# leo-stan/torch-points3d

Hardware: AMD Instinct MI355X
Metric: point-clouds/sec fwd+bwd PointNet++SSG B=32 N=16384 (higher is better)
Workload: dtype f32; 1 GPU; PointNet++ SSG (unet_3_ss) train step fwd+bwd+Adam, B=32 per GPU, N=16384, FEAT=3, 10 classes, pos~U[-1,1]^3 (BASELINE configs[1]); launch=hip-graph replay; geometry of step i+1 on a 2nd stream during step i, global_batch=32, points=16384, parallelism=dp1, whole clouds per rank, one flat gradient all-reduce (RCCL) per step

## Files before the change

### torch_points3d_amd/csrc/rows.hip

```cpp
#include "tp3d_common.h"

namespace tp3d {

constexpr int RW_BLOCK = 256;

__global__ __launch_bounds__(RW_BLOCK) void group_concat_fwd_kernel(const float *__restrict__ pos,
                                                                     const float *__restrict__ new_pos,
                                                                     const float *__restrict__ x_cl,
                                                                     const int64_t *__restrict__ idx, int N, int np,
                                                                     int ns, int C, int ld, float radius,
                                                                     int normalize, int64_t total,
                                                                     float *__restrict__ out)
{
    const int Cw = C + 3;
    for (int64_t e = (int64_t)blockIdx.x * RW_BLOCK + threadIdx.x; e < total; e += (int64_t)gridDim.x * RW_BLOCK) {
        const int64_t row = e / ld;
        const int c = (int)(e - row * ld);
        if (c >= Cw) {
            out[e] = 0.0f;
            continue;
        }
        const int64_t bj = row / ns;
        const int b = (int)(bj / np);
        const int k = min(max((int)idx[row], 0), N - 1);
        float v;
        if (c < 3) {
            v = pos[((size_t)b * N + k) * 3 + c] - new_pos[bj * 3 + c];
            if (normalize) v = v / radius;
        } else {
            v = x_cl[((size_t)b * N + k) * C + (c - 3)];
        }
        out[e] = v;
    }
}

struct __attribute__((packed, aligned(4))) f4u {
    float v[4];
};
__global__ __launch_bounds__(RW_BLOCK) void group_concat_fwd4_kernel(const float *__restrict__ pos,
                                                                      const float *__restrict__ new_pos,
                                                                      const float *__restrict__ x_cl,
                                                                      const int64_t *__restrict__ idx, int N, int np,
                                                                      int ns, int C, int ld, float radius,
                                                                      int normalize, int64_t total4,
                                                                      float *__restrict__ out)
{
    const int Cw = C + 3, q = ld >> 2;
    for (int64_t e4 = (int64_t)blockIdx.x * RW_BLOCK + threadIdx.x; e4 < total4; e4 += (int64_t)gridDim.x * RW_BLOCK) {
        const int64_t row = e4 / q;
        const int c = (int)(e4 - row * q) * 4;
        const int64_t bj = row / ns;
        const int b = (int)(bj / np);
        const int k = min(max((int)idx[row], 0), N - 1);
        float t[4];
        if (c == 0) {
#pragma unroll
            for (int j = 0; j < 3; ++j) {
                float v = pos[((size_t)b * N + k) * 3 + j] - new_pos[bj * 3 + j];
                if (normalize) v = v / radius;
                t[j] = v;
            }
            t[3] = C > 0 ? x_cl[((size_t)b * N + k) * C] : 0.0f;
        } else if (c + 3 < Cw) {
            const f4u f = *reinterpret_cast<const f4u *>(x_cl + ((size_t)b * N + k) * C + (c - 3));
#pragma unroll
            for (int j = 0; j < 4; ++j) t[j] = f.v[j];
        } else {
#pragma unroll
            for (int j = 0; j < 4; ++j) t[j] = (c + j < Cw) ? x_cl[((size_t)b * N + k) * C + (c + j - 3)] : 0.0f;
        }
        *reinterpret_cast<float4 *>(out + e4 * 4) = make_float4(t[0], t[1], t[2], t[3]);
    }
}

constexpr int ST_ROWS = 256;
constexpr int ST_ROWS_SMALL = 32;
constexpr int64_t ST_SMALL_BELOW = 131072;
static inline int stat_rows(int64_t R) { return R >= ST_SMALL_BELOW ? ST_ROWS : ST_ROWS_SMALL; }

struct StatTile {
    int colthreads, rowlanes, gridx;
};
static inline StatTile stat_tile(int C, int V)
{
    int cols = (C + V - 1) / V;
    int ct = 1;
    while (ct < cols && ct < 64) ct <<= 1;
    StatTile t;
    t.colthreads = ct;
    t.rowlanes = RW_BLOCK / ct;
    t.gridx = (cols + ct - 1) / ct;
    return t;
}

template <int V, int MODE>
__global__ __launch_bounds__(RW_BLOCK) void colreduce_partial_kernel(
    const float *__restrict__ Y, const float *__restrict__ dA, const float *__restrict__ scale,
    const float *__restrict__ shift, const float *__restrict__ mean, const float *__restrict__ invstd, float slope,
    int64_t M, int C, int colthreads, int chunk_rows, float *__restrict__ partial , int reverse = 0)
{
    __shared__ float s1[RW_BLOCK * V], s2[RW_BLOCK * V];
    const int ct = threadIdx.x % colthreads, rl = threadIdx.x / colthreads;
    const int rowlanes = RW_BLOCK / colthreads;
    const int c = (blockIdx.x * colthreads + ct) * V;
    const int chunk = (MODE == 1 && reverse) ? (int)(gridDim.y - 1 - blockIdx.y) : (int)blockIdx.y;
    const int64_t r0 = (int64_t)chunk * chunk_rows;
    const int64_t r1 = min(r0 + chunk_rows, M);
    float a[V], q[V], sc[V], sh[V], mu[V], is[V];
#pragma unroll
    for (int v = 0; v < V; ++v) {
        a[v] = 0.0f;
        q[v] = 0.0f;
        if (MODE == 0) mu[v] = (c + v < C && r0 < M) ? Y[r0 * C + c + v] : 0.0f;
        if (MODE == 1 && c + v < C) {
            sc[v] = scale[c + v];
            sh[v] = shift[c + v];
            mu[v] = mean[c + v];
            is[v] = invstd[c + v];
        }
    }
    if (c < C) {
        constexpr int U = 4;
        for (int64_t r = r0 + rl; r < r1; r += (int64_t)rowlanes * U) {
            float y[U][V], d[U][V];
// ... 234 lines not shown
            o.y = leaky((y.y - mu.y) * sc.y + sh.y, slope);
            o.z = leaky((y.z - mu.z) * sc.z + sh.z, slope);
            o.w = leaky((y.w - mu.w) * sc.w + sh.w, slope);
            *reinterpret_cast<float4 *>(out + e) = o;
        } else {
            out[e] = leaky((Y[e] - mean[cw.c]) * scale[cw.c] + shift[cw.c], slope);
        }
    }
}

__global__ __launch_bounds__(RW_BLOCK) void bn_act_maxpool_kernel(const float *__restrict__ Y,
                                                                   const float *__restrict__ mean,
                                                                   const float *__restrict__ scale,
                                                                   const float *__restrict__ shift, float slope,
                                                                   int64_t G, int ns, int C,
                                                                   float *__restrict__ out, int *__restrict__ arg)
{
    const int64_t total = G * C;
    for (int64_t e = (int64_t)blockIdx.x * RW_BLOCK + threadIdx.x; e < total; e += (int64_t)gridDim.x * RW_BLOCK) {
        const int64_t g = e / C;
        const int c = (int)(e - g * C);
        const float mu = mean[c], sc = scale[c], sh = shift[c];
        const float *y = Y + (size_t)g * ns * C + c;
        float best = -INFINITY;
        int bs = 0;
        int s = 0;
        auto take = [&](float a, int row) {
            const bool is_nan = (__float_as_uint(a) & 0x7fffffffu) > 0x7f800000u;
            const bool have_nan = (__float_as_uint(best) & 0x7fffffffu) > 0x7f800000u;
            if (!have_nan && (is_nan || a > best)) {
                best = a;
                bs = row;
            }
        };
        for (; s + 8 <= ns; s += 8) {
            float v[8];
#pragma unroll
            for (int u = 0; u < 8; ++u) v[u] = y[(size_t)(s + u) * C];
#pragma unroll
            for (int u = 0; u < 8; ++u) {
                const float z = (v[u] - mu) * sc + sh;
                take(z > 0.0f ? z : z * slope, s + u);
            }
        }
        for (; s < ns; ++s) {
            const float z = (y[(size_t)s * C] - mu) * sc + sh;
            take(z > 0.0f ? z : z * slope, s);
        }
        out[e] = best;
        arg[e] = bs;
    }
}

__global__ __launch_bounds__(RW_BLOCK) void bn_pool_bwd_partial_kernel(const float *__restrict__ dP,
                                                                        const int *__restrict__ arg,
                                                                        const float *__restrict__ Y,
                                                                        const float *__restrict__ scale,
                                                                        const float *__restrict__ shift,
                                                                        const float *__restrict__ mean,
                                                                        const float *__restrict__ invstd, float slope,
                                                                        int64_t G, int ns, int C, int chunk_rows,
                                                                        float *__restrict__ partial)
{
    __shared__ float s1[4][64], s2[4][64];
    const int tc = threadIdx.x & 63, tr = threadIdx.x >> 6;
    const int c = blockIdx.x * 64 + tc;
    const int64_t g0 = (int64_t)blockIdx.y * chunk_rows;
    const int64_t g1 = min(g0 + chunk_rows, G);
    float a = 0.0f, q = 0.0f;
    if (c < C) {
        const float sc = scale[c], sh = shift[c], mu = mean[c], is = invstd[c];
        for (int64_t g = g0 + tr; g < g1; g += 4) {
            const int s = arg[g * C + c];
            const float y = Y[((size_t)g * ns + s) * C + c];
            const float z = (y - mu) * sc + sh;
            const float dz = dP[g * C + c] * (z > 0.0f ? 1.0f : slope);
            a += dz;
            q += dz * ((y - mu) * is);
        }
    }
    s1[tr][tc] = a;
    s2[tr][tc] = q;
    __syncthreads();
    if (tr == 0 && c < C) {
        a = (s1[0][tc] + s1[1][tc]) + (s1[2][tc] + s1[3][tc]);
        q = (s2[0][tc] + s2[1][tc]) + (s2[2][tc] + s2[3][tc]);
        partial[((size_t)blockIdx.y * 2 + 0) * C + c] = a;
        partial[((size_t)blockIdx.y * 2 + 1) * C + c] = q;
    }
}

__global__ __launch_bounds__(RW_BLOCK) void bn_bwd_finalize_kernel(const float *__restrict__ partial, int chunks,
                                                                    int C, float *__restrict__ dbeta,
                                                                    float *__restrict__ dgamma,
                                                                    const float *__restrict__ invstd, int64_t M,
                                                                    int training, float *__restrict__ c1,
                                                                    float *__restrict__ c2)
{
    double a, q;
    sum_partials(partial, chunks, C, blockIdx.x, a, q);
    if (threadIdx.x == 0) {
        dbeta[blockIdx.x] = (float)a;
        dgamma[blockIdx.x] = (float)q;
        if (c1) {
            const float invM = 1.0f / (float)M;
            c1[blockIdx.x] = training ? (float)a * invM : 0.0f;
            c2[blockIdx.x] = training ? invstd[blockIdx.x] * ((float)q * invM) : 0.0f;
        }
    }
}

__device__ __forceinline__ float bn_bwd_elem(float da, float y, float sc, float sh, float mu, float is, float db,
                                             float dg, float slope, float invM, int training)
{
    const float z = (y - mu) * sc + sh;
    const float dz = da * (z > 0.0f ? 1.0f : slope);
    float v = dz;
    if (training) v = dz - db * invM - ((y - mu) * is) * (dg * invM);
    return sc * v;
}

template <int V>
__global__ __launch_bounds__(RW_BLOCK) void bn_act_bwd_apply_kernel(
    const float *__restrict__ dA, const float *__restrict__ Y, const float *__restrict__ scale,
    const float *__restrict__ shift, const float *__restrict__ mean, const float *__restrict__ invstd,
    const float *__restrict__ dbeta, const float *__restrict__ dgamma, float slope, int64_t M, int C, int training,
    float *__restrict__ dY)
{
    const int64_t total = M * C;
    const float invM = 1.0f / (float)M;
    const int64_t stride = (int64_t)gridDim.x * RW_BLOCK * V;
// ... 69 lines not shown
        const size_t base = (size_t)g * ns * C + c;
        const int s_end = min(ns, (seg + 1) * seg_len);
        int s = seg * seg_len;
        for (; s + 8 <= s_end; s += 8) {
            float y[8];
#pragma unroll
            for (int u = 0; u < 8; ++u) y[u] = Y[base + (size_t)(s + u) * C];
#pragma unroll
            for (int u = 0; u < 8; ++u)
                dY[base + (size_t)(s + u) * C] =
                    bn_bwd_elem(s + u == sa ? dp : 0.0f, y[u], sc, sh, mu, is, db, dg, slope, invM, training);
        }
        for (; s < s_end; ++s) {
            const float y = Y[base + (size_t)s * C];
            dY[base + (size_t)s * C] = bn_bwd_elem(s == sa ? dp : 0.0f, y, sc, sh, mu, is, db, dg, slope, invM, training);
        }
    }
}

__global__ __launch_bounds__(RW_BLOCK) void interp_concat_fwd_kernel(const float *__restrict__ feat_cl,
                                                                      const int64_t *__restrict__ idx,
                                                                      const float *__restrict__ w,
                                                                      const float *__restrict__ skip_cl, int m, int n,
                                                                      int C1, int C2, int ld, int64_t total,
                                                                      float *__restrict__ out)
{
    const int Cw = C1 + C2;
    for (int64_t e = (int64_t)blockIdx.x * RW_BLOCK + threadIdx.x; e < total; e += (int64_t)gridDim.x * RW_BLOCK) {
        const int64_t row = e / ld;
        const int c = (int)(e - row * ld);
        if (c >= Cw) {
            out[e] = 0.0f;
            continue;
        }
        float v;
        if (c < C1) {
            const int b = (int)(row / n);
            const int64_t *ip = idx + row * 3;
            const float *wp = w + row * 3;
            const int k0 = min(max((int)ip[0], 0), m - 1), k1 = min(max((int)ip[1], 0), m - 1),
                      k2 = min(max((int)ip[2], 0), m - 1);
            const float *fb = feat_cl + (size_t)b * m * C1 + c;
            const float a0 = wp[0] * fb[(size_t)k0 * C1];
            const float a1 = wp[1] * fb[(size_t)k1 * C1];
            const float a2 = wp[2] * fb[(size_t)k2 * C1];
            v = (a0 + a1) + a2;
        } else {
            v = skip_cl[row * C2 + (c - C1)];
        }
        out[e] = v;
    }
}

__global__ __launch_bounds__(RW_BLOCK) void interp_concat_fwd4_kernel(const float *__restrict__ feat_cl,
                                                                       const int64_t *__restrict__ idx,
                                                                       const float *__restrict__ w,
                                                                       const float *__restrict__ skip_cl, int m, int n,
                                                                       int C1, int C2, int ld, int64_t total4,
                                                                       float *__restrict__ out)
{
    const int Cw = C1 + C2, q = ld >> 2;
    for (int64_t e4 = (int64_t)blockIdx.x * RW_BLOCK + threadIdx.x; e4 < total4; e4 += (int64_t)gridDim.x * RW_BLOCK) {
        const int64_t row = e4 / q;
        const int c = (int)(e4 - row * q) * 4;
        float4 v;
        if (c < C1) {
            const int b = (int)(row / n);
            const int64_t *ip = idx + row * 3;
            const float *wp = w + row * 3;
            const int k0 = min(max((int)ip[0], 0), m - 1), k1 = min(max((int)ip[1], 0), m - 1),
                      k2 = min(max((int)ip[2], 0), m - 1);
            const float w0 = wp[0], w1 = wp[1], w2 = wp[2];
            const float *fb = feat_cl + (size_t)b * m * C1 + c;
            const float4 f0 = *reinterpret_cast<const float4 *>(fb + (size_t)k0 * C1);
            const float4 f1 = *reinterpret_cast<const float4 *>(fb + (size_t)k1 * C1);
            const float4 f2 = *reinterpret_cast<const float4 *>(fb + (size_t)k2 * C1);
            v.x = (w0 * f0.x + w1 * f1.x) + w2 * f2.x;
            v.y = (w0 * f0.y + w1 * f1.y) + w2 * f2.y;
            v.z = (w0 * f0.z + w1 * f1.z) + w2 * f2.z;
            v.w = (w0 * f0.w + w1 * f1.w) + w2 * f2.w;
        } else {
            float t[4];
#pragma unroll
            for (int j = 0; j < 4; ++j) t[j] = (c + j < Cw) ? skip_cl[row * C2 + (c + j - C1)] : 0.0f;
            v = make_float4(t[0], t[1], t[2], t[3]);
        }
        *reinterpret_cast<float4 *>(out + e4 * 4) = v;
    }
}

__global__ void idw_weights_kernel(const float *__restrict__ dist, int64_t rows, float *__restrict__ w)
{
    const int64_t r = (int64_t)blockIdx.x * blockDim.x + threadIdx.x;
    if (r >= rows) return;
    const float r0 = 1.0f / (dist[r * 3 + 0] + 1e-8f);
    const float r1 = 1.0f / (dist[r * 3 + 1] + 1e-8f);
    const float r2 = 1.0f / (dist[r * 3 + 2] + 1e-8f);
    const float norm = (r0 + r1) + r2;
    w[r * 3 + 0] = r0 / norm;
    w[r * 3 + 1] = r1 / norm;
    w[r * 3 + 2] = r2 / norm;
}

static inline unsigned grid_for(int64_t total)
{
    int64_t g = (total + RW_BLOCK - 1) / RW_BLOCK;
    return (unsigned)(g < 1 ? 1 : (g > 8192 ? 8192 : g));
}

}

using namespace tp3d;

TP3D_EXPORT int tp3d_group_concat_fwd_f32(const float *pos, const float *new_pos, const float *x_cl,
                                          const int64_t *idx, int B, int N, int np, int ns, int C, int ld,
                                          float radius, int normalize, float *out, void *stream)
{
    if (B < 0 || N <= 0 || np < 0 || ns < 0 || C < 0 || ld < C + 3) return TP3D_E_BADARG;
    const int64_t total = (int64_t)B * np * ns * ld;
    if (total == 0) return TP3D_OK;
    if (!pos || !new_pos || !idx || !out || (C > 0 && !x_cl)) return TP3D_E_BADARG;
    if ((ld & 3) == 0 && ((uintptr_t)out & 15) == 0)
        hipLaunchKernelGGL(group_concat_fwd4_kernel, dim3(grid_for(total / 4)), dim3(RW_BLOCK), 0, (hipStream_t)stream,
                           pos, new_pos, x_cl, idx, N, np, ns, C, ld, radius, normalize, total / 4, out);
    else
        hipLaunchKernelGGL(group_concat_fwd_kernel, dim3(grid_for(total)), dim3(RW_BLOCK), 0, (hipStream_t)stream, pos,
                           new_pos, x_cl, idx, N, np, ns, C, ld, radius, normalize, total, out);
    return check_launch();
}

TP3D_EXPORT size_t tp3d_bn_workspace_floats(int64_t M, int C)
{
    if (M < 0 || C < 0) return 0;
    int64_t chunks = M >= ST_SMALL_BELOW ? (M + ST_ROWS - 1) / ST_ROWS : (M + ST_ROWS_SMALL - 1) / ST_ROWS_SMALL;
    if (M >= ST_SMALL_BELOW && chunks < ST_SMALL_BELOW / ST_ROWS_SMALL) chunks = ST_SMALL_BELOW / ST_ROWS_SMALL;
    return (size_t)chunks * 4 * (size_t)C;
}

TP3D_EXPORT int tp3d_bn_plan(int64_t M, int C, int pooled_ns, int64_t *plan)
{
    if (M <= 0 || C <= 0 || pooled_ns < 0 || !plan) return TP3D_E_BADARG;
    const int64_t R = pooled_ns > 1 ? M / pooled_ns : M;
    const int crow = stat_rows(R);
    plan[0] = crow;
    plan[1] = (R + crow - 1) / crow;
    plan[2] = plan[1] * (pooled_ns == 0 ? 4 : 2) * C;
    return TP3D_OK;
}

constexpr int BN_DIRECT_CHUNKS = 64, BN_SLICES = 32;
static int launch_bn_finalize(float *partial, int chunks, int64_t M, int C, float eps, float momentum, const float *gamma,
                              const float *beta, float *running_mean, float *running_var, int64_t *batches, int training,
                              float *mean, float *invstd, float *scale, float *shift, hipStream_t s)
{
    int n = chunks, stride = 1;
    if (training && chunks > BN_DIRECT_CHUNKS) {
        stride = (chunks + BN_SLICES - 1) / BN_SLICES;
        n = (chunks + stride - 1) / stride;
        hipLaunchKernelGGL(bn_merge_slices_kernel, dim3((C + BM_COLS - 1) / BM_COLS, n), dim3(RW_BLOCK), 0, s, partial, chunks,
                           stride, C);
        if (int rc = check_launch()) return rc;
    }
    hipLaunchKernelGGL(bn_finalize_kernel, dim3(C), dim3(RW_BLOCK), 0, s, partial, n, stride, M, C, eps, momentum, gamma, beta,
                       running_mean, running_var, batches, training, mean, invstd, scale, shift);
    return check_launch();
}

TP3D_EXPORT int tp3d_bn_stats_f32(const float *Y, int64_t M, int C, float eps, float momentum, const float *gamma,
                                  const float *beta, float *running_mean, float *running_var,
                                  int64_t *num_batches_tracked, int training, float *mean, float *invstd, float *scale,
                                  float *shift, float *workspace, void *stream)
{
    if (M <= 0 || C <= 0 || !mean || !invstd || !scale || !shift) return TP3D_E_BADARG;
    if (!training && (!running_mean || !running_var)) return TP3D_E_BADARG;
    hipStream_t s = (hipStream_t)stream;
    const int crow = stat_rows(M);
    const int chunks = (int)((M + crow - 1) / crow);
    if (training) {
        if (!Y || !workspace) return TP3D_E_BADARG;
        if (chunks > 65535) return TP3D_E_TOOBIG;
        if ((C & 3) == 0) {
            const StatTile t = stat_tile(C, 4);
            hipLaunchKernelGGL((colreduce_partial_kernel<4, 0>), dim3(t.gridx, chunks), dim3(RW_BLOCK), 0, s, Y,
                               (const float *)nullptr, (const float *)nullptr, (const float *)nullptr,
                               (const float *)nullptr, (const float *)nullptr, 0.0f, M, C, t.colthreads, crow, workspace);
        } else {
            const StatTile t = stat_tile(C, 1);
            hipLaunchKernelGGL((colreduce_partial_kernel<1, 0>), dim3(t.gridx, chunks), dim3(RW_BLOCK), 0, s, Y,
                               (const float *)nullptr, (const float *)nullptr, (const float *)nullptr,
                               (const float *)nullptr, (const float *)nullptr, 0.0f, M, C, t.colthreads, crow, workspace);
        }
        if (int rc = check_launch()) return rc;
    }
    return launch_bn_finalize(workspace, chunks, M, C, eps, momentum, gamma, beta, running_mean, running_var,
                              num_batches_tracked, training, mean, invstd, scale, shift, s);
}

TP3D_EXPORT int tp3d_bn_finalize_f32(float *partial, int chunks, int64_t M, int C, float eps, float momentum,
                                     const float *gamma, const float *beta, float *running_mean, float *running_var,
                                     int64_t *num_batches_tracked, float *mean, float *invstd, float *scale, float *shift,
                                     void *stream)
{
    if (M <= 0 || C <= 0 || chunks <= 0 || !partial || !mean || !invstd || !scale || !shift) return TP3D_E_BADARG;
    return launch_bn_finalize(partial, chunks, M, C, eps, momentum, gamma, beta, running_mean, running_var,
                              num_batches_tracked, 1, mean, invstd, scale, shift, (hipStream_t)stream);
}

TP3D_EXPORT int tp3d_bn_act_f32(const float *Y, const float *mean, const float *scale, const float *shift, float slope,
                                int64_t M, int C, float *out, void *stream)
{
    if (M < 0 || C <= 0) return TP3D_E_BADARG;
    if (M == 0) return TP3D_OK;
    if (!Y || !mean || !scale || !shift || !out) return TP3D_E_BADARG;
    const int64_t total = M * C;
    if ((C & 3) == 0)
        hipLaunchKernelGGL(bn_act_kernel<4>, dim3(grid_for(total / 4)), dim3(RW_BLOCK), 0, (hipStream_t)stream, Y, mean,
                           scale, shift, slope, total, C, out);
    else
        hipLaunchKernelGGL(bn_act_kernel<1>, dim3(grid_for(total)), dim3(RW_BLOCK), 0, (hipStream_t)stream, Y, mean,
                           scale, shift, slope, total, C, out);
    return check_launch();
}

TP3D_EXPORT int tp3d_bn_act_maxpool_f32(const float *Y, const float *mean, const float *scale, const float *shift,
                                        float slope, int64_t G, int ns, int C, float *out, int *argmax, void *stream)
{
    if (G < 0 || ns <= 0 || C <= 0) return TP3D_E_BADARG;
    if (G == 0) return TP3D_OK;
    if (!Y || !mean || !scale || !shift || !out || !argmax) return TP3D_E_BADARG;
    hipLaunchKernelGGL(bn_act_maxpool_kernel, dim3(grid_for(G * C)), dim3(RW_BLOCK), 0, (hipStream_t)stream, Y, mean, scale,
                       shift, slope, G, ns, C, out, argmax);
    return check_launch();
}

namespace tp3d {
int bn_bwd_finalize_launch(const float *partial, int chunks, int C, float *dbeta, float *dgamma, const float *invstd, int64_t M,
                           int training, float *c1, float *c2, hipStream_t s)
{
    hipLaunchKernelGGL(bn_bwd_finalize_kernel, dim3(C), dim3(RW_BLOCK), 0, s, partial, chunks, C, dbeta, dgamma, invstd, M,
                       training, c1, c2);
    return check_launch();
}

static int bn_bwd_reduce(const float *dA, const int *argmax, const float *Y, const float *scale, const float *shift,
                         const float *mean, const float *invstd, float slope, int64_t M, int ns, int C, int training,
                         float *dbeta, float *dgamma, float *c1, float *c2, float *workspace, int reverse, hipStream_t s)
{
    const int64_t R = argmax ? M / ns : M;
    const int crow = stat_rows(R);
    const int chunks = (int)((R + crow - 1) / crow);
    if (chunks > 65535) return TP3D_E_TOOBIG;
    if (argmax) {
        hipLaunchKernelGGL(bn_pool_bwd_partial_kernel, dim3((C + 63) / 64, chunks), dim3(RW_BLOCK), 0, s, dA, argmax, Y,
                           scale, shift, mean, invstd, slope, R, ns, C, crow, workspace);
    } else if ((C & 3) == 0) {
        const StatTile t = stat_tile(C, 4);
        hipLaunchKernelGGL((colreduce_partial_kernel<4, 1>), dim3(t.gridx, chunks), dim3(RW_BLOCK), 0, s, Y, dA, scale,
                           shift, mean, invstd, slope, M, C, t.colthreads, crow, workspace, reverse);
    } else {
        const StatTile t = stat_tile(C, 1);
        hipLaunchKernelGGL((colreduce_partial_kernel<1, 1>), dim3(t.gridx, chunks), dim3(RW_BLOCK), 0, s, Y, dA, scale,
                           shift, mean, invstd, slope, M, C, t.colthreads, crow, workspace);
    }
    if (int rc = check_launch()) return rc;
    hipLaunchKernelGGL(bn_bwd_finalize_kernel, dim3(C), dim3(RW_BLOCK), 0, s, workspace, chunks, C, dbeta, dgamma, invstd, M,
                       training, c1, c2);
    return check_launch();
}
}

TP3D_EXPORT int tp3d_bn_bwd_reduce_f32(const float *dA, const int *argmax, const float *Y, const float *scale,
                                       const float *shift, const float *mean, const float *invstd, float slope,
                                       int64_t M, int ns, int C, int training, float *dbeta, float *dgamma, float *c1,
                                       float *c2, float *workspace, int reverse, void *stream)
{
    if (M <= 0 || C <= 0 || ns <= 0 || (argmax && M % ns)) return TP3D_E_BADARG;
    if (!dA || !Y || !scale || !shift || !mean || !invstd || !dbeta || !dgamma || !c1 || !c2 || !workspace)
        return TP3D_E_BADARG;
    return bn_bwd_reduce(dA, argmax, Y, scale, shift, mean, invstd, slope, M, ns, C, training, dbeta, dgamma, c1, c2,
                         workspace, reverse, (hipStream_t)stream);
}

TP3D_EXPORT int tp3d_bn_act_bwd_f32(const float *dA, const int *argmax, const float *Y, const float *scale,
                                    const float *shift, const float *mean, const float *invstd, float slope,
                                    int64_t M, int ns, int C, int training, float *dbeta, float *dgamma, float *dY,
                                    float *workspace, void *stream)
{
    if (M <= 0 || C <= 0 || ns <= 0 || (argmax && M % ns)) return TP3D_E_BADARG;
    if (!dA || !Y || !scale || !shift || !mean || !invstd || !dbeta || !dgamma || !dY || !workspace)
        return TP3D_E_BADARG;
    hipStream_t s = (hipStream_t)stream;
    const int64_t R = argmax ? M / ns : M;
    if (int rc = bn_bwd_reduce(dA, argmax, Y, scale, shift, mean, invstd, slope, M, ns, C, training, dbeta, dgamma, nullptr,
                               nullptr, workspace, 0, s))
        return rc;
    if (argmax) {
        int split = (int)((262144 + R * C - 1) / (R * C));
        split = split < 1 ? 1 : (split > ns ? ns : split);
        hipLaunchKernelGGL(bn_pool_bwd_apply_kernel, dim3(grid_for(R * C * split)), dim3(RW_BLOCK), 0, s, dA, argmax, Y,
                           scale, shift, mean, invstd, dbeta, dgamma, slope, R, ns, C, split, training, dY);
    }
    else if ((C & 3) == 0)
        hipLaunchKernelGGL(bn_act_bwd_apply_kernel<4>, dim3(grid_for(M * C / 4)), dim3(RW_BLOCK), 0, s, dA, Y, scale,
                           shift, mean, invstd, dbeta, dgamma, slope, M, C, training, dY);
    else
        hipLaunchKernelGGL(bn_act_bwd_apply_kernel<1>, dim3(grid_for(M * C)), dim3(RW_BLOCK), 0, s, dA, Y, scale,
                           shift, mean, invstd, dbeta, dgamma, slope, M, C, training, dY);
    return check_launch();
}

TP3D_EXPORT int tp3d_interp_concat_fwd_f32(const float *feat_cl, const int64_t *idx, const float *weight,
                                           const float *skip_cl, int B, int m, int n, int C1, int C2, int ld,
                                           float *out, void *stream)
{
    if (B < 0 || m <= 0 || n < 0 || C1 < 0 || C2 < 0 || ld < C1 + C2) return TP3D_E_BADARG;
    const int64_t total = (int64_t)B * n * ld;
    if (total == 0) return TP3D_OK;
    if (!out || (C1 > 0 && (!feat_cl || !idx || !weight)) || (C2 > 0 && !skip_cl)) return TP3D_E_BADARG;
    if ((ld & 3) == 0 && (C1 & 3) == 0 && (((uintptr_t)feat_cl | (uintptr_t)out) & 15) == 0)
        hipLaunchKernelGGL(interp_concat_fwd4_kernel, dim3(grid_for(total / 4)), dim3(RW_BLOCK), 0, (hipStream_t)stream,
                           feat_cl, idx, weight, skip_cl, m, n, C1, C2, ld, total / 4, out);
    else
        hipLaunchKernelGGL(interp_concat_fwd_kernel, dim3(grid_for(total)), dim3(RW_BLOCK), 0, (hipStream_t)stream,
                           feat_cl, idx, weight, skip_cl, m, n, C1, C2, ld, total, out);
    return check_launch();
}

namespace tp3d {
__global__ __launch_bounds__(RW_BLOCK) void relation_rows_kernel(const float *__restrict__ pos,
                                                                  const float *__restrict__ new_pos,
                                                                  const int64_t *__restrict__ idx, int N, int np, int ns,
                                                                  int ld, int64_t rows, float *__restrict__ out)
{
    for (int64_t row = (int64_t)blockIdx.x * RW_BLOCK + threadIdx.x; row < rows; row += (int64_t)gridDim.x * RW_BLOCK) {
        const int64_t bj = row / ns;
        const int b = (int)(bj / np);
        const int k = min(max((int)idx[row], 0), N - 1);
        const float *p = pos + ((size_t)b * N + k) * 3, *c = new_pos + bj * 3;
        const float px = p[0], py = p[1], pz = p[2], cx = c[0], cy = c[1], cz = c[2];
        const float dx = px - cx, dy = py - cy, dz = pz - cz;
        float v[12] = {sqrtf((dx * dx + dy * dy) + dz * dz), cx, cy, cz, px, py, pz, dx, dy, dz, 0.0f, 0.0f};
        float *o = out + row * ld;
        if (ld == 12 && ((uintptr_t)out & 15) == 0) {
#pragma unroll
            for (int q = 0; q < 3; ++q) reinterpret_cast<float4 *>(o)[q] = make_float4(v[4 * q], v[4 * q + 1], v[4 * q + 2], v[4 * q + 3]);
        } else {
            for (int q = 0; q < ld; ++q) o[q] = q < 10 ? v[q] : 0.0f;
        }
    }
}
}

TP3D_EXPORT int tp3d_relation_rows_f32(const float *pos, const float *new_pos, const int64_t *idx, int B, int N, int np,
                                       int ns, int ld, float *out, void *stream)
{
    if (B < 0 || N <= 0 || np < 0 || ns < 0 || ld < 10) return TP3D_E_BADARG;
    const int64_t rows = (int64_t)B * np * ns;
    if (rows == 0) return TP3D_OK;
    if (!pos || !new_pos || !idx || !out) return TP3D_E_BADARG;
    hipLaunchKernelGGL(relation_rows_kernel, dim3(grid_for(rows)), dim3(RW_BLOCK), 0, (hipStream_t)stream, pos, new_pos, idx,
                       N, np, ns, ld, rows, out);
    return check_launch();
}

TP3D_EXPORT int tp3d_idw_weights_f32(const float *dist, int64_t rows, float *weight, void *stream)
{
    if (rows < 0) return TP3D_E_BADARG;
    if (rows == 0) return TP3D_OK;
    if (!dist || !weight) return TP3D_E_BADARG;
    hipLaunchKernelGGL(idw_weights_kernel, dim3((unsigned)((rows + 255) / 256)), dim3(256), 0, (hipStream_t)stream,
                       dist, rows, weight);
    return check_launch();
}
```

### torch_points3d_amd/csrc/run_sum.hip

```cpp
#include <type_traits>

#include "inverse_table.h"

namespace tp3d {

constexpr int RW_BLOCK = 256;

__device__ __forceinline__ float rl_f(float x, int lane)
{
    return __builtin_bit_cast(float, __builtin_amdgcn_readlane(__builtin_bit_cast(int, x), lane));
}

template <int NP>
__device__ __forceinline__ void gather_run(const float *__restrict__ base, const int *__restrict__ od,
                                           const float *__restrict__ ws, int lo, int hi, int ld, const int (&c)[NP],
                                           float (&acc)[NP], int lane)
{
    for (int j0 = lo; j0 < hi; j0 += 64) {
        const int cnt = min(64, hi - j0);
        const int my_r = (lane < cnt) ? od[j0 + lane] : 0;
        const float my_w = (ws && lane < cnt) ? ws[j0 + lane] : 1.0f;
        int t = 0;
        auto take = [&](auto utag) {
            constexpr int U = decltype(utag)::value;
            int r[U];
            float wv[U], v[U][NP];
#pragma unroll
            for (int u = 0; u < U; ++u) {
                r[u] = __builtin_amdgcn_readlane(my_r, t + u);
                wv[u] = ws ? rl_f(my_w, t + u) : 1.0f;
            }
#pragma unroll
            for (int u = 0; u < U; ++u)
#pragma unroll
                for (int p = 0; p < NP; ++p) v[u][p] = base[(size_t)r[u] * ld + c[p]];
#pragma unroll
            for (int u = 0; u < U; ++u)
#pragma unroll
                for (int p = 0; p < NP; ++p) acc[p] = acc[p] + (ws ? wv[u] * v[u][p] : v[u][p]);
            t += U;
        };
        while (t + 8 <= cnt) take(std::integral_constant<int, 8>());
        if (t + 4 <= cnt) take(std::integral_constant<int, 4>());
        const int rem = cnt - t;
        if (rem > 0) {
            const int r0 = __builtin_amdgcn_readlane(my_r, t);
            const int r1 = __builtin_amdgcn_readlane(my_r, min(t + 1, cnt - 1));
            const int r2 = __builtin_amdgcn_readlane(my_r, min(t + 2, cnt - 1));
            const float w0 = ws ? rl_f(my_w, t) : 1.0f, w1 = ws ? rl_f(my_w, min(t + 1, cnt - 1)) : 1.0f,
                        w2 = ws ? rl_f(my_w, min(t + 2, cnt - 1)) : 1.0f;
#pragma unroll
            for (int p = 0; p < NP; ++p) {
                const float v0 = base[(size_t)r0 * ld + c[p]], v1 = base[(size_t)r1 * ld + c[p]],
                            v2 = base[(size_t)r2 * ld + c[p]];
                acc[p] = acc[p] + (ws ? w0 * v0 : v0);
                if (rem > 1) acc[p] = acc[p] + (ws ? w1 * v1 : v1);
                if (rem > 2) acc[p] = acc[p] + (ws ? w2 * v2 : v2);
            }
        }
    }
}

constexpr int HUB_MIN = 128;
constexpr int HUB_BLOCK = 1024;

template <int NP>
__global__ __launch_bounds__(RW_BLOCK) void rows_gather_sum_kernel(const float *__restrict__ grad_rows,
                                                                    const int *__restrict__ start,
                                                                    const int *__restrict__ order,
                                                                    const float *__restrict__ wsorted, int nbins,
                                                                    int L, int rows_per_cloud, int ld, int col0,
                                                                    int C, float *__restrict__ out, int flat, int hub_min)
{
    const int lane = threadIdx.x & 63;
    const int64_t dest = (int64_t)blockIdx.x * (RW_BLOCK / 64) + (threadIdx.x >> 6);
    const int b = blockIdx.y;
    if (dest >= nbins) return;
    const int *st = flat ? start + (size_t)b * nbins : start + (size_t)b * (nbins + 1);
    const int *od = flat ? order : order + (size_t)b * L;
    const float *ws = wsorted ? (flat ? wsorted : wsorted + (size_t)b * L) : nullptr;
    const int lo = st[dest], hi = st[dest + 1];
    if (hub_min > 0 && hi - lo > hub_min) return;
    const float *base = grad_rows + (flat ? (size_t)0 : (size_t)b * rows_per_cloud * ld) + col0;
    for (int c0 = 0; c0 < C; c0 += 64 * NP) {
        int c[NP];
        float acc[NP];
#pragma unroll
        for (int p = 0; p < NP; ++p) {
            c[p] = min(c0 + p * 64 + lane, C - 1);
            acc[p] = 0.0f;
        }
        gather_run<NP>(base, od, ws, lo, hi, ld, c, acc, lane);
#pragma unroll
        for (int p = 0; p < NP; ++p)
            if (c0 + p * 64 + lane < C) out[((size_t)b * nbins + dest) * C + c0 + p * 64 + lane] = acc[p];
    }
}

__global__ __launch_bounds__(256) void find_hubs_kernel(const int *__restrict__ start, int B, int nbins, int flat,
                                                        int *__restrict__ hubs)
{
    const int64_t e = (int64_t)blockIdx.x * 256 + threadIdx.x;
    if (e >= (int64_t)B * nbins) return;
    const int b = (int)(e / nbins), k = (int)(e - (int64_t)b * nbins);
    const int *st = flat ? start + (size_t)b * nbins : start + (size_t)b * (nbins + 1);
    if (st[k + 1] - st[k] > HUB_MIN) hubs[1 + atomicAdd(&hubs[0], 1)] = (int)e;
}

template <int NP>
__global__ __launch_bounds__(HUB_BLOCK) void rows_gather_hub_kernel(const float *__restrict__ grad_rows,
                                                                     const int *__restrict__ start,
                                                                     const int *__restrict__ order,
                                                                     const float *__restrict__ wsorted,
                                                                     const int *__restrict__ hubs, int nbins, int L,
                                                                     int rows_per_cloud, int ld, int col0, int C,
                                                                     float *__restrict__ out, int flat)
{
    constexpr int NW = HUB_BLOCK / 64;
    __shared__ float part[NW][64 * NP];
    const int lane = threadIdx.x & 63, wave = threadIdx.x >> 6;
    const int count = hubs[0];
    for (int h = blockIdx.x; h < count; h += gridDim.x) {
        const int e = hubs[1 + h];
        const int b = e / nbins, dest = e - b * nbins;
        const int *st = flat ? start + (size_t)b * nbins : start + (size_t)b * (nbins + 1);
        const int *od = flat ? order : order + (size_t)b * L;
        const float *ws = wsorted ? (flat ? wsorted : wsorted + (size_t)b * L) : nullptr;
        const int lo = st[dest], hi = st[dest + 1];
        const int per = ((hi - lo + NW - 1) / NW + 7) & ~7;
        const int wlo = min(lo + wave * per, hi), whi = min(wlo + per, hi);
        const float *base = grad_rows + (flat ? (size_t)0 : (size_t)b * rows_per_cloud * ld) + col0;
        for (int c0 = 0; c0 < C; c0 += 64 * NP) {
            int c[NP];
            float acc[NP];
#pragma unroll
            for (int p = 0; p < NP; ++p) {
                c[p] = min(c0 + p * 64 + lane, C - 1);
                acc[p] = 0.0f;
            }
            gather_run<NP>(base, od, ws, wlo, whi, ld, c, acc, lane);
#pragma unroll
            for (int p = 0; p < NP; ++p) part[wave][p * 64 + lane] = acc[p];
            __syncthreads();
            for (int x = threadIdx.x; x < 64 * NP; x += HUB_BLOCK) {
                float sum = part[0][x];
                for (int w = 1; w < NW; ++w) sum = sum + part[w][x];
                const int cc = c0 + x;
                if (cc < C) out[((size_t)b * nbins + dest) * C + cc] = sum;
            }
            __syncthreads();
        }
    }
}

template <typename F>
static void with_np(int C, F f)
{
    if (C > 128) f(std::integral_constant<int, 4>());
    else if (C > 64) f(std::integral_constant<int, 2>());
    else f(std::integral_constant<int, 1>());
}

int find_hubs(const int *start, int B, int nbins, bool flat, int *hubs, hipStream_t s)
{
    if (int rc = zero_async(hubs, sizeof(int), s)) return rc;
    hipLaunchKernelGGL(find_hubs_kernel, dim3((unsigned)(((int64_t)B * nbins + 255) / 256)), dim3(256), 0, s, start, B, nbins,
                       flat ? 1 : 0, hubs);
    return check_launch();
}

int gather_slot_rows(const float *g, const int *start, const int *order, int64_t M, int Cin, float *d_x, hipStream_t s)
{
    const dim3 grid((unsigned)((M + RW_BLOCK / 64 - 1) / (RW_BLOCK / 64)));
    with_np(Cin, [&](auto np) {
        hipLaunchKernelGGL(rows_gather_sum_kernel<decltype(np)::value>, grid, dim3(RW_BLOCK), 0, s, g, start, order, nullptr,
                           (int)M, 0, 0, Cin, 0, Cin, d_x, 1, 0);
    });
    return check_launch();
}

constexpr int GS_BLOCK = 512;
constexpr int GS_HUB_MIN = 128;
// ... 181 lines not shown
```

Before: 4222 point-clouds/s.

## Rework gather-concat, interp-concat, maxpool and hub gather kernels for row-wise access

The group-concat and interp-concat forward kernels become wave-per-row-block kernels that fetch indices once per lane and broadcast them with shuffles. Consecutive lanes then cover the columns of a row, which should improve coalescing and cut per-element index loads. A new 4-channel vectorised BN+activation+maxpool kernel, optionally splitting ns across waves, replaces the scalar one when alignment allows. The BN pool backward loop is unrolled to batch its loads. The scatter-gather gains a 16-wide unroll, and mid-sized hubs are handled inline with piecewise summation that matches the hub kernel's reduction order, while only large hubs go to the hub kernel. This adds code complexity and several template variants.

Result: no change. 4229 point-clouds/s (median of 6 runs) (+0.2%).

```diff
diff --git a/torch_points3d_amd/csrc/rows.hip b/torch_points3d_amd/csrc/rows.hip
--- a/torch_points3d_amd/csrc/rows.hip
+++ b/torch_points3d_amd/csrc/rows.hip
@@ -1,3 +1,5 @@
+#include <type_traits>
+
 #include "tp3d_common.h"
 
 namespace tp3d {
@@ -34,42 +36,69 @@
     }
 }
 
-struct __attribute__((packed, aligned(4))) f4u {
-    float v[4];
-};
-__global__ __launch_bounds__(RW_BLOCK) void group_concat_fwd4_kernel(const float *__restrict__ pos,
+constexpr int CC_U = 4;
+static inline int lanes_per_row(int units, int least)
+{
+    int l = least;
+    while (l < units && l < 64) l <<= 1;
+    return l;
+}
+static inline unsigned row_grid(int64_t rows, int rows_per_wave)
+{
+    const int64_t waves = (rows + rows_per_wave - 1) / rows_per_wave;
+    const int64_t g = (waves + RW_BLOCK / 64 - 1) / (RW_BLOCK / 64);
+    return (unsigned)(g < 1 ? 1 : (g > 16384 ? 16384 : g));
+}
+
+template <int LPR>
+__global__ __launch_bounds__(RW_BLOCK) void group_concat_fwd_rows_kernel(const float *__restrict__ pos,
                                                                       const float *__restrict__ new_pos,
                                                                       const float *__restrict__ x_cl,
                                                                       const int64_t *__restrict__ idx, int N, int np,
                                                                       int ns, int C, int ld, float radius,
-                                                                      int normalize, int64_t total4,
-                                                                      float *__restrict__ out)
-{
-    const int Cw = C + 3, q = ld >> 2;
-    for (int64_t e4 = (int64_t)blockIdx.x * RW_BLOCK + threadIdx.x; e4 < total4; e4 += (int64_t)gridDim.x * RW_BLOCK) {
-        const int64_t row = e4 / q;
-        const int c = (int)(e4 - row * q) * 4;
-        const int64_t bj = row / ns;
-        const int b = (int)(bj / np);
-        const int k = min(max((int)idx[row], 0), N - 1);
-        float t[4];
-        if (c == 0) {
-#pragma unroll
-            for (int j = 0; j < 3; ++j) {
-                float v = pos[((size_t)b * N + k) * 3 + j] - new_pos[bj * 3 + j];
-                if (normalize) v = v / radius;
-                t[j] = v;
-            }
-            t[3] = C > 0 ? x_cl[((size_t)b * N + k) * C] : 0.0f;
-        } else if (c + 3 < Cw) {
-            const f4u f = *reinterpret_cast<const f4u *>(x_cl + ((size_t)b * N + k) * C + (c - 3));
-#pragma unroll
-            for (int j = 0; j < 4; ++j) t[j] = f.v[j];
-        } else {
-#pragma unroll
-            for (int j = 0; j < 4; ++j) t[j] = (c + j < Cw) ? x_cl[((size_t)b * N + k) * C + (c + j - 3)] : 0.0f;
-        }
-        *reinterpret_cast<float4 *>(out + e4 * 4) = make_float4(t[0], t[1], t[2], t[3]);
+                                                                      int normalize, int rows, float *__restrict__ out)
+{
+    constexpr int RPP = 64 / LPR, RB = CC_U * RPP;
+    const int lane = threadIdx.x & 63, sub = lane / LPR, cl = lane % LPR;
+    const int Cw = C + 3;
+    const int64_t wave = (int64_t)blockIdx.x * (RW_BLOCK / 64) + (threadIdx.x >> 6);
+    const int64_t step = (int64_t)gridDim.x * (RW_BLOCK / 64) * RB;
+    for (int64_t row0 = wave * RB; row0 < rows; row0 += step) {
+        const int r0 = (int)row0;
+        int g = 0, bj = 0;
+        if (lane < RB && r0 + lane < rows) {
+            bj = (r0 + lane) / ns;
+            g = (bj / np) * N + min(max((int)idx[r0 + lane], 0), N - 1);
+        }
+        int gi[CC_U], bji[CC_U];
+#pragma unroll
+        for (int u = 0; u < CC_U; ++u) {
+            gi[u] = __shfl(g, u * RPP + sub);
+            bji[u] = __shfl(bj, u * RPP + sub);
+        }
+        for (int c0 = 0; c0 < ld; c0 += LPR) {
+            const int c = c0 + cl;
+            const bool xyz = c < 3, feat = !xyz && c < Cw;
+            float a[CC_U], cen[CC_U];
+#pragma unroll
+            for (int u = 0; u < CC_U; ++u) {
+                const float *src = feat ? x_cl + (size_t)gi[u] * C + (c - 3) : pos + (size_t)gi[u] * 3 + min(c, 2);
+                a[u] = *src;
+                cen[u] = 0.0f;
+            }
+            if (c0 == 0) {
+#pragma unroll
+                for (int u = 0; u < CC_U; ++u) cen[u] = new_pos[(size_t)bji[u] * 3 + min(c, 2)];
+            }
+#pragma unroll
+            for (int u = 0; u < CC_U; ++u) {
+                float d = a[u] - cen[u];
+                if (normalize) d = d / radius;
+                const float v = xyz ? d : (feat ? a[u] : 0.0f);
+                const int r = r0 + u * RPP + sub;
+                if (c < ld && r < rows) out[(size_t)r * ld + c] = v;
+            }
+        }
     }
 }
 
@@ -410,6 +439,88 @@
     }
 }
 
+constexpr int64_t POOL_SPLIT_BELOW = 131072;
+constexpr int POOL_SPLIT_ROWS = 32;
+template <bool SPLIT>
+__global__ __launch_bounds__(RW_BLOCK) void bn_act_maxpool_kernel_quads(const float *__restrict__ Y,
+                                                                    const float *__restrict__ mean,
+                                                                    const float *__restrict__ scale,
+                                                                    const float *__restrict__ shift, float slope,
+                                                                    int64_t G, int ns, int C, float *__restrict__ out,
+                                                                    int *__restrict__ arg)
+{
+    constexpr int PARTS = SPLIT ? RW_BLOCK / 64 : 1, ITEMS = RW_BLOCK / PARTS;
+    __shared__ float s_best[PARTS][4][64];
+    __shared__ int s_row[PARTS][4][64];
+    const int Q = C >> 2;
+    const int64_t items = G * Q;
+    const int part = SPLIT ? (int)(threadIdx.x >> 6) : 0, slot = SPLIT ? (int)(threadIdx.x & 63) : (int)threadIdx.x;
+    const int seg = (ns + PARTS - 1) / PARTS;
+    const int s0 = min(part * seg, ns), s1 = min(s0 + seg, ns);
+    for (int64_t i0 = (int64_t)blockIdx.x * ITEMS; i0 < items; i0 += (int64_t)gridDim.x * ITEMS) {
+        const int64_t e = i0 + slot;
+        const bool live = e < items;
+        float best[4] = {-INFINITY, -INFINITY, -INFINITY, -INFINITY};
+        int bs[4] = {0, 0, 0, 0};
+        auto take = [&](int j, float a, int row) {
+            const bool is_nan = (__float_as_uint(a) & 0x7fffffffu) > 0x7f800000u;
+            const bool have_nan = (__float_as_uint(best[j]) & 0x7fffffffu) > 0x7f800000u;
+            const bool upd = !have_nan && (is_nan || a > best[j]);
+            best[j] = upd ? a : best[j];
+            bs[j] = upd ? row : bs[j];
+        };
+        if (live) {
+            const int64_t g = e / Q;
+            const int c = (int)(e - g * Q) * 4;
+            float mu[4], sc[4], sh[4];
+            *reinterpret_cast<float4 *>(mu) = *reinterpret_cast<const float4 *>(mean + c);
+            *reinterpret_cast<float4 *>(sc) = *reinterpret_cast<const float4 *>(scale + c);
+            *reinterpret_cast<float4 *>(sh) = *reinterpret_cast<const float4 *>(shift + c);
+            const float *y = Y + (size_t)g * ns * C + c;
+            int s = s0;
+            for (; s + 8 <= s1; s += 8) {
+                float v[8][4];
+#pragma unroll
+                for (int u = 0; u < 8; ++u)
+                    *reinterpret_cast<float4 *>(v[u]) = *reinterpret_cast<const float4 *>(y + (size_t)(s + u) * C);
+#pragma unroll
+                for (int u = 0; u < 8; ++u)
+#pragma unroll
+                    for (int j = 0; j < 4; ++j) {
+                        const float z = (v[u][j] - mu[j]) * sc[j] + sh[j];
+                        take(j, z > 0.0f ? z : z * slope, s + u);
+                    }
+            }
+            for (; s < s1; ++s) {
+                float v[4];
+                *reinterpret_cast<float4 *>(v) = *reinterpret_cast<const float4 *>(y + (size_t)s * C);
+#pragma unroll
+                for (int j = 0; j < 4; ++j) {
+                    const float z = (v[j] - mu[j]) * sc[j] + sh[j];
+                    take(j, z > 0.0f ? z : z * slope, s);
+                }
+            }
+        }
+        if (SPLIT) {
+#pragma unroll
+            for (int j = 0; j < 4; ++j) {
+                s_best[part][j][slot] = best[j];
+                s_row[part][j][slot] = bs[j];
+            }
+            __syncthreads();
+            if (part == 0)
+                for (int p = 1; p < PARTS; ++p)
+#pragma unroll
+                    for (int j = 0; j < 4; ++j) take(j, s_best[p][j][slot], s_row[p][j][slot]);
+            __syncthreads();
+        }
+        if (live && part == 0) {
+            *reinterpret_cast<float4 *>(out + e * 4) = make_float4(best[0], best[1], best[2], best[3]);
+            *reinterpret_cast<int4 *>(arg + e * 4) = make_int4(bs[0], bs[1], bs[2], bs[3]);
+        }
+    }
+}
+
 __global__ __launch_bounds__(RW_BLOCK) void bn_pool_bwd_partial_kernel(const float *__restrict__ dP,
                                                                         const int *__restrict__ arg,
                                                                         const float *__restrict__ Y,
@@ -428,13 +539,30 @@
     float a = 0.0f, q = 0.0f;
     if (c < C) {
         const float sc = scale[c], sh = shift[c], mu = mean[c], is = invstd[c];
-        for (int64_t g = g0 + tr; g < g1; g += 4) {
-            const int s = arg[g * C + c];
-            const float y = Y[((size_t)g * ns + s) * C + c];
-            const float z = (y - mu) * sc + sh;
-            const float dz = dP[g * C + c] * (z > 0.0f ? 1.0f : slope);
-            a += dz;
-            q += dz * ((y - mu) * is);
+        constexpr int U = 8;
+        for (int64_t g = g0 + tr; g < g1; g += 4 * U) {
+            int s[U];
+            float dp[U], y[U];
+#pragma unroll
+            for (int u = 0; u < U; ++u) {
+                const int64_t gg = g + 4 * u;
+                s[u] = gg < g1 ? arg[gg * C + c] : 0;
+                dp[u] = gg < g1 ? dP[gg * C + c] : 0.0f;
+            }
+#pragma unroll
+            for (int u = 0; u < U; ++u) {
+                const int64_t gg = g + 4 * u;
+                y[u] = gg < g1 ? Y[((size_t)gg * ns + s[u]) * C + c] : 0.0f;
+            }
+#pragma unroll
+            for (int u = 0; u < U; ++u) {
+                if (g + 4 * u < g1) {
+                    const float z = (y[u] - mu) * sc + sh;
+                    const float dz = dp[u] * (z > 0.0f ? 1.0f : slope);
+                    a += dz;
+                    q += dz * ((y[u] - mu) * is);
+                }
+            }
         }
     }
     s1[tr][tc] = a;
@@ -610,40 +738,59 @@
     }
 }
 
-__global__ __launch_bounds__(RW_BLOCK) void interp_concat_fwd4_kernel(const float *__restrict__ feat_cl,
+template <int LPR>
+__global__ __launch_bounds__(RW_BLOCK) void interp_concat_fwd_rows_kernel(const float *__restrict__ feat_cl,
                                                                        const int64_t *__restrict__ idx,
                                                                        const float *__restrict__ w,
                                                                        const float *__restrict__ skip_cl, int m, int n,
-                                                                       int C1, int C2, int ld, int64_t total4,
+                                                                       int C1, int C2, int ld, int rows,
                                                                        float *__restrict__ out)
 {
-    const int Cw = C1 + C2, q = ld >> 2;
-    for (int64_t e4 = (int64_t)blockIdx.x * RW_BLOCK + threadIdx.x; e4 < total4; e4 += (int64_t)gridDim.x * RW_BLOCK) {
-        const int64_t row = e4 / q;
-        const int c = (int)(e4 - row * q) * 4;
-        float4 v;
-        if (c < C1) {
-            const int b = (int)(row / n);
-            const int64_t *ip = idx + row * 3;
-            const float *wp = w + row * 3;
-            const int k0 = min(max((int)ip[0], 0), m - 1), k1 = min(max((int)ip[1], 0), m - 1),
-                      k2 = min(max((int)ip[2], 0), m - 1);
-            const float w0 = wp[0], w1 = wp[1], w2 = wp[2];
-            const float *fb = feat_cl + (size_t)b * m * C1 + c;
-            const float4 f0 = *reinterpret_cast<const float4 *>(fb + (size_t)k0 * C1);
-            const float4 f1 = *reinterpret_cast<const float4 *>(fb + (size_t)k1 * C1);
-            const float4 f2 = *reinterpret_cast<const float4 *>(fb + (size_t)k2 * C1);
-            v.x = (w0 * f0.x + w1 * f1.x) + w2 * f2.x;
-            v.y = (w0 * f0.y + w1 * f1.y) + w2 * f2.y;
-            v.z = (w0 * f0.z + w1 * f1.z) + w2 * f2.z;
-            v.w = (w0 * f0.w + w1 * f1.w) + w2 * f2.w;
-        } else {
+    constexpr int RPP = 64 / LPR, RB = CC_U * RPP;
+    static_assert(3 * RB <= 64, "the (index, weight) triples of a wave step are fetched by one lane each");
+    const int lane = threadIdx.x & 63, sub = lane / LPR, cl = lane % LPR;
+    const int Cw = C1 + C2, fq = C1 >> 2, tq = (ld >> 2) - fq;
+    const int64_t wave = (int64_t)blockIdx.x * (RW_BLOCK / 64) + (threadIdx.x >> 6);
+    const int64_t step = (int64_t)gridDim.x * (RW_BLOCK / 64) * RB;
+    for (int64_t row0 = wave * RB; row0 < rows; row0 += step) {
+        const int r0 = (int)row0;
+        int g = 0;
+        float wt = 0.0f;
+        if (fq > 0 && lane < 3 * RB && r0 + lane / 3 < rows) {
+            g = ((r0 + lane / 3) / n) * m + min(max((int)idx[(int64_t)r0 * 3 + lane], 0), m - 1);
+            wt = w[(int64_t)r0 * 3 + lane];
+        }
+        for (int cq0 = 0; cq0 < fq; cq0 += LPR) {
+            const int cq = min(cq0 + cl, fq - 1);
+            float4 f[CC_U][3];
+            float ww[CC_U][3];
+#pragma unroll
+            for (int u = 0; u < CC_U; ++u)
+#pragma unroll
+                for (int t = 0; t < 3; ++t) {
+                    const int src = 3 * (u * RPP + sub) + t;
+                    ww[u][t] = __shfl(wt, src);
+                    f[u][t] = *reinterpret_cast<const float4 *>(feat_cl + (size_t)__shfl(g, src) * C1 + cq * 4);
+                }
+#pragma unroll
+            for (int u = 0; u < CC_U; ++u) {
+                const int r = r0 + u * RPP + sub;
+                float4 v;
+                v.x = (ww[u][0] * f[u][0].x + ww[u][1] * f[u][1].x) + ww[u][2] * f[u][2].x;
+                v.y = (ww[u][0] * f[u][0].y + ww[u][1] * f[u][1].y) + ww[u][2] * f[u][2].y;
+                v.z = (ww[u][0] * f[u][0].z + ww[u][1] * f[u][1].z) + ww[u][2] * f[u][2].z;
+                v.w = (ww[u][0] * f[u][0].w + ww[u][1] * f[u][1].w) + ww[u][2] * f[u][2].w;
+                if (cq0 + cl < fq && r < rows) *reinterpret_cast<float4 *>(out + (size_t)r * ld + cq * 4) = v;
+            }
+        }
+        for (int i = lane; i < RB * tq; i += 64) {
+            const int rl = i / tq, c = (fq + (i - rl * tq)) * 4, r = r0 + rl;
+            if (r >= rows) break;
             float t[4];
 #pragma unroll
-            for (int j = 0; j < 4; ++j) t[j] = (c + j < Cw) ? skip_cl[row * C2 + (c + j - C1)] : 0.0f;
-            v = make_float4(t[0], t[1], t[2], t[3]);
-        }
-        *reinterpret_cast<float4 *>(out + e4 * 4) = v;
+            for (int j = 0; j < 4; ++j) t[j] = (c + j < Cw) ? skip_cl[(int64_t)r * C2 + (c + j - C1)] : 0.0f;
+            *reinterpret_cast<float4 *>(out + (size_t)r * ld + c) = make_float4(t[0], t[1], t[2], t[3]);
+        }
     }
 }
 
@@ -678,10 +825,21 @@
     const int64_t total = (int64_t)B * np * ns * ld;
     if (total == 0) return TP3D_OK;
     if (!pos || !new_pos || !idx || !out || (C > 0 && !x_cl)) return TP3D_E_BADARG;
-    if ((ld & 3) == 0 && ((uintptr_t)out & 15) == 0)
-        hipLaunchKernelGGL(group_concat_fwd4_kernel, dim3(grid_for(total / 4)), dim3(RW_BLOCK), 0, (hipStream_t)stream,
-                           pos, new_pos, x_cl, idx, N, np, ns, C, ld, radius, normalize, total / 4, out);
-    else
+    const int64_t rows = total / ld;
+    if ((ld & 3) == 0 && ((uintptr_t)out & 15) == 0 && rows < INT32_MAX / 4 && (int64_t)B * N < INT32_MAX) {
+        auto launch = [&](auto lpr) {
+            constexpr int LPR = decltype(lpr)::value;
+            hipLaunchKernelGGL(group_concat_fwd_rows_kernel<LPR>, dim3(row_grid(rows, CC_U * 64 / LPR)), dim3(RW_BLOCK), 0,
+                               (hipStream_t)stream, pos, new_pos, x_cl, idx, N, np, ns, C, ld, radius, normalize, (int)rows,
+                               out);
+        };
+        switch (lanes_per_row(ld, 8)) {
+        case 8: launch(std::integral_constant<int, 8>()); break;
+        case 16: launch(std::integral_constant<int, 16>()); break;
+        case 32: launch(std::integral_constant<int, 32>()); break;
+        default: launch(std::integral_constant<int, 64>()); break;
+        }
+    } else
         hipLaunchKernelGGL(group_concat_fwd_kernel, dim3(grid_for(total)), dim3(RW_BLOCK), 0, (hipStream_t)stream, pos,
                            new_pos, x_cl, idx, N, np, ns, C, ld, radius, normalize, total, out);
     return check_launch();
@@ -786,8 +944,18 @@
     if (G < 0 || ns <= 0 || C <= 0) return TP3D_E_BADARG;
     if (G == 0) return TP3D_OK;
     if (!Y || !mean || !scale || !shift || !out || !argmax) return TP3D_E_BADARG;
-    hipLaunchKernelGGL(bn_act_maxpool_kernel, dim3(grid_for(G * C)), dim3(RW_BLOCK), 0, (hipStream_t)stream, Y, mean, scale,
-                       shift, slope, G, ns, C, out, argmax);
+    const bool quads = (C & 3) == 0 && (((uintptr_t)Y | (uintptr_t)mean | (uintptr_t)scale | (uintptr_t)shift | (uintptr_t)out |
+                                         (uintptr_t)argmax) & 15) == 0;
+    const int64_t items = G * (C >> 2);
+    if (quads && items < POOL_SPLIT_BELOW && ns >= POOL_SPLIT_ROWS)
+        hipLaunchKernelGGL(bn_act_maxpool_kernel_quads<true>, dim3(grid_for(items * (RW_BLOCK / 64))), dim3(RW_BLOCK), 0,
+                           (hipStream_t)stream, Y, mean, scale, shift, slope, G, ns, C, out, argmax);
+    else if (quads)
+        hipLaunchKernelGGL(bn_act_maxpool_kernel_quads<false>, dim3(grid_for(items)), dim3(RW_BLOCK), 0, (hipStream_t)stream, Y,
+                           mean, scale, shift, slope, G, ns, C, out, argmax);
+    else
+        hipLaunchKernelGGL(bn_act_maxpool_kernel, dim3(grid_for(G * C)), dim3(RW_BLOCK), 0, (hipStream_t)stream, Y, mean,
+                           scale, shift, slope, G, ns, C, out, argmax);
     return check_launch();
 }
 
@@ -875,10 +1043,20 @@
     const int64_t total = (int64_t)B * n * ld;
     if (total == 0) return TP3D_OK;
     if (!out || (C1 > 0 && (!feat_cl || !idx || !weight)) || (C2 > 0 && !skip_cl)) return TP3D_E_BADARG;
-    if ((ld & 3) == 0 && (C1 & 3) == 0 && (((uintptr_t)feat_cl | (uintptr_t)out) & 15) == 0)
-        hipLaunchKernelGGL(interp_concat_fwd4_kernel, dim3(grid_for(total / 4)), dim3(RW_BLOCK), 0, (hipStream_t)stream,
-                           feat_cl, idx, weight, skip_cl, m, n, C1, C2, ld, total / 4, out);
-    else
+    const int64_t rows = (int64_t)B * n;
+    if ((ld & 3) == 0 && (C1 & 3) == 0 && (((uintptr_t)feat_cl | (uintptr_t)out) & 15) == 0 && rows < INT32_MAX / 4 &&
+        (int64_t)B * m < INT32_MAX) {
+        auto launch = [&](auto lpr) {
+            constexpr int LPR = decltype(lpr)::value;
+            hipLaunchKernelGGL(interp_concat_fwd_rows_kernel<LPR>, dim3(row_grid(rows, CC_U * 64 / LPR)), dim3(RW_BLOCK), 0,
+                               (hipStream_t)stream, feat_cl, idx, weight, skip_cl, m, n, C1, C2, ld, (int)rows, out);
+        };
+        switch (lanes_per_row(C1 >> 2, 16)) {
+        case 16: launch(std::integral_constant<int, 16>()); break;
+        case 32: launch(std::integral_constant<int, 32>()); break;
+        default: launch(std::integral_constant<int, 64>()); break;
+        }
+    } else
         hipLaunchKernelGGL(interp_concat_fwd_kernel, dim3(grid_for(total)), dim3(RW_BLOCK), 0, (hipStream_t)stream,
                            feat_cl, idx, weight, skip_cl, m, n, C1, C2, ld, total, out);
     return check_launch();
diff --git a/torch_points3d_amd/csrc/run_sum.hip b/torch_points3d_amd/csrc/run_sum.hip
--- a/torch_points3d_amd/csrc/run_sum.hip
+++ b/torch_points3d_amd/csrc/run_sum.hip
@@ -40,7 +40,8 @@
                 for (int p = 0; p < NP; ++p) acc[p] = acc[p] + (ws ? wv[u] * v[u][p] : v[u][p]);
             t += U;
         };
-        while (t + 8 <= cnt) take(std::integral_constant<int, 8>());
+        while (t + 16 <= cnt) take(std::integral_constant<int, 16>());
+        if (t + 8 <= cnt) take(std::integral_constant<int, 8>());
         if (t + 4 <= cnt) take(std::integral_constant<int, 4>());
         const int rem = cnt - t;
         if (rem > 0) {
@@ -61,7 +62,64 @@
     }
 }
 
+constexpr int HUB_PIECES = 16;
+__host__ __device__ __forceinline__ int hub_piece_slots(int len) { return ((len + HUB_PIECES - 1) / HUB_PIECES + 7) & ~7; }
+
+template <int NP>
+__device__ __forceinline__ void gather_pieces(const float *__restrict__ base, const int *__restrict__ od,
+                                              const float *__restrict__ ws, int lo, int hi, int ld, const int (&c)[NP],
+                                              float (&total)[NP], int lane)
+{
+    const int per = hub_piece_slots(hi - lo);
+    float acc[NP];
+#pragma unroll
+    for (int p = 0; p < NP; ++p) acc[p] = 0.0f;
+    int piece = 0, left = per;
+    auto fold = [&]() {
+#pragma unroll
+        for (int p = 0; p < NP; ++p) {
+            total[p] = piece == 0 ? acc[p] : total[p] + acc[p];
+            acc[p] = 0.0f;
+        }
+        ++piece;
+        left = per;
+    };
+    for (int j0 = lo; j0 < hi; j0 += 64) {
+        const int cnt = min(64, hi - j0);
+        const int my_r = (lane < cnt) ? od[j0 + lane] : 0;
+        const float my_w = (ws && lane < cnt) ? ws[j0 + lane] : 1.0f;
+        for (int t = 0; t < cnt;) {
+            const int nb = min(min(8, left), cnt - t);
+            int r[8];
+            float wv[8], v[8][NP];
+#pragma unroll
+            for (int u = 0; u < 8; ++u) {
+                const int src = t + min(u, nb - 1);
+                r[u] = __builtin_amdgcn_readlane(my_r, src);
+                wv[u] = ws ? rl_f(my_w, src) : 1.0f;
+            }
+#pragma unroll
+            for (int u = 0; u < 8; ++u)
+#pragma unroll
+                for (int p = 0; p < NP; ++p) v[u][p] = base[(size_t)r[u] * ld + c[p]];
+#pragma unroll
+            for (int u = 0; u < 8; ++u)
+                if (u < nb)
+#pragma unroll
+                    for (int p = 0; p < NP; ++p) acc[p] = acc[p] + (ws ? wv[u] * v[u][p] : v[u][p]);
+            t += nb;
+            left -= nb;
+            if (left == 0) fold();
+        }
+    }
+    if (left < per) fold();
+    for (; piece < HUB_PIECES; ++piece)
+#pragma unroll
+        for (int p = 0; p < NP; ++p) total[p] = total[p] + 0.0f;
+}
+
 constexpr int HUB_MIN = 128;
+constexpr int HUB_INLINE = 256;
 constexpr int HUB_BLOCK = 1024;
 
 template <int NP>
@@ -79,8 +137,9 @@
     const int *st = flat ? start + (size_t)b * nbins : start + (size_t)b * (nbins + 1);
     const int *od = flat ? order : order + (size_t)b * L;
     const float *ws = wsorted ? (flat ? wsorted : wsorted + (size_t)b * L) : nullptr;
-    const int lo = st[dest], hi = st[dest + 1];
-    if (hub_min > 0 && hi - lo > hub_min) return;
+    const int lo = __builtin_amdgcn_readfirstlane(st[dest]), hi = __builtin_amdgcn_readfirstlane(st[dest + 1]);
+    const bool pieces = hub_min > 0 && hi - lo > hub_min;
+    if (pieces && hi - lo > HUB_INLINE) return;
     const float *base = grad_rows + (flat ? (size_t)0 : (size_t)b * rows_per_cloud * ld) + col0;
     for (int c0 = 0; c0 < C; c0 += 64 * NP) {
         int c[NP];
@@ -90,7 +149,8 @@
             c[p] = min(c0 + p * 64 + lane, C - 1);
             acc[p] = 0.0f;
         }
-        gather_run<NP>(base, od, ws, lo, hi, ld, c, acc, lane);
+        if (pieces) gather_pieces<NP>(base, od, ws, lo, hi, ld, c, acc, lane);
+        else gather_run<NP>(base, od, ws, lo, hi, ld, c, acc, lane);
 #pragma unroll
         for (int p = 0; p < NP; ++p)
             if (c0 + p * 64 + lane < C) out[((size_t)b * nbins + dest) * C + c0 + p * 64 + lane] = acc[p];
@@ -117,6 +177,7 @@
                                                                      float *__restrict__ out, int flat)
 {
     constexpr int NW = HUB_BLOCK / 64;
+    static_assert(NW == HUB_PIECES, "one wave per piece");
     __shared__ float part[NW][64 * NP];
     const int lane = threadIdx.x & 63, wave = threadIdx.x >> 6;
     const int count = hubs[0];
@@ -127,7 +188,8 @@
         const int *od = flat ? order : order + (size_t)b * L;
         const float *ws = wsorted ? (flat ? wsorted : wsorted + (size_t)b * L) : nullptr;
         const int lo = st[dest], hi = st[dest + 1];
-        const int per = ((hi - lo + NW - 1) / NW + 7) & ~7;
+        if (hi - lo <= HUB_INLINE) continue;
+        const int per = hub_piece_slots(hi - lo);
         const int wlo = min(lo + wave * per, hi), whi = min(wlo + per, hi);
         const float *base = grad_rows + (flat ? (size_t)0 : (size_t)b * rows_per_cloud * ld) + col0;
         for (int c0 = 0; c0 < C; c0 += 64 * NP) {
```
